# linto-ai/ssak

Measured on AMD Instinct MI355X. Metric: utterances/sec (16 kHz, 10 s) Wav2Vec2-base CTC train step, higher is better.
Workload: dtype bf16; 1 GPU; Wav2Vec2-base CTC fine-tune step, bf16, synthetic 10 s @16 kHz utterances (BASELINE.json configs[1]; DP over xGMI for n_gpus>1 = configs[2]); per_gpu_batch=32, global_batch=32, samples_per_utt=160000, frames=499, frozen_feature_encoder=True, regularisers=script defaults (dropout/layerdrop/specaugment on), parallelism=dp1

## Files before the change

ssak_amd/csrc/kernels.h:

```cpp
#pragma once
#include "common.h"

enum : int {
  PROF_ATTN_FWD = 0, PROF_ATTN_BWD, PROF_LN_FWD, PROF_LN_BWD, PROF_CONV0, PROF_ADAMW, PROF_SUMSQ, PROF_CTC, PROF_WAVE_NORM,
  PROF_ROWWISE, PROF_POSCONV_W, PROF_SOFTMAX, PROF_POSCONV_DIRECT, PROF_POSCONV_WGRAD, PROF_LOGMEL,
  PROF_CLASS_SLOTS
};
constexpr int PROF_MAX_SLOTS = 128;
int ssak_prof_register(const char* name, int bound);
bool ssak_prof_wanted(int slot, hipStream_t st);
class ProfScope {
 public:
  ProfScope(int slot, double work, hipStream_t st);
  ~ProfScope();
  ProfScope(const ProfScope&) = delete;
  ProfScope& operator=(const ProfScope&) = delete;

 private:
  hipStream_t st_;
  hipEvent_t e0_ = nullptr;
  int slot_;
  double work_;
  bool on_;
};

struct DropSpec {
  uint64_t seed = 0;
  uint32_t stream = 0;
  float p = 0.f;
};

struct ReduceJob {
  const float* partial;
  float* out;
  long stride;
  int slots, ncols;
};
struct ReduceSink {
  static constexpr int CAP = 32;
  ReduceJob jobs[CAP];
  int n = 0;
  bool push(const float* partial, long stride, int slots, int ncols, float* out) {
    if (n >= CAP) return false;
    jobs[n++] = ReduceJob{partial, out, stride, slots, ncols};
    return true;
  }
};
extern thread_local ReduceSink* g_reduce_sink;
int k_reduce_flush(ReduceSink& sink, hipStream_t st);

template <typename T>
int k_layernorm_fwd_t(const T* y, const T* res, const float* gamma, const float* beta, T* r_out, T* out,
                      float* mean, float* rstd, int M, int C, float eps, const DropSpec& pre, const DropSpec& post,
                      hipStream_t st, const DropSpec& mid = DropSpec(), bool post_gelu = false);
template <typename T>
int k_layernorm_bwd_t(const T* g1, const T* g2, const T* r, const float* mean, const float* rstd,
                      const float* gamma, const T* g_res, T* dr, T* dy, float* dgamma, float* dbeta,
                      float* partial , int M, int C, const DropSpec& pre, const DropSpec& post,
                      hipStream_t st, const DropSpec& mid = DropSpec(), float* dy_colsum = nullptr ,
                      const float* post_gelu_beta = nullptr );
#ifndef SSAK_LN_BWD_BLOCKS
#define SSAK_LN_BWD_BLOCKS 768
#endif
#ifndef SSAK_LN_FWD_BLOCKS
#define SSAK_LN_FWD_BLOCKS 768
#endif
constexpr int LN_FWD_BLOCKS = SSAK_LN_FWD_BLOCKS;
constexpr int LN_BWD_BLOCKS = SSAK_LN_BWD_BLOCKS;
template <typename T>
int k_softmax_fwd_t(const T* S, T* P, T* Pd, const int32_t* klens, int rows, int cols, int ld,
                    int rows_per_batch, const DropSpec& drop, hipStream_t st);
template <typename T>
int k_softmax_bwd_t(const T* dPd, const T* P, T* dS, int rows, int cols, int ld, const DropSpec& drop,
                    hipStream_t st);
template <typename T>
int k_colsum_t(const T* X, long ld, int M, int N, float* out, hipStream_t st, float* scratch = nullptr, size_t scratch_floats = 0,
               const uint8_t* rowmask = nullptr, const int32_t* flens = nullptr, int F = 0);
int k_cast_f32_bf16(const float* in, bf16* out, long n, hipStream_t st);
template <typename T>
int k_specaug_fwd_t(T* h, const uint8_t* mask, const int32_t* flens, const float* embed, int B, int F, int C,
                    hipStream_t st);
template <typename T>
int k_specaug_bwd_t(T* dh, const uint8_t* mask, const int32_t* flens, float* dembed, int B, int F, int C,
                    hipStream_t st, float* scratch = nullptr, size_t scratch_floats = 0);
template <typename T>
int k_gelu_grad_mul_t(const T* dy, const T* pre, T* out, long n, hipStream_t st);
template <typename T>
int k_add_t(const T* a, const T* b, T* out, long n, hipStream_t st);
int k_layernorm_fwd(const bf16* y, const bf16* res, const float* gamma, const float* beta, bf16* r_out, bf16* out,
                    float* mean, float* rstd, int M, int C, float eps, const DropSpec& pre, const DropSpec& post,
                    hipStream_t st, const DropSpec& mid = DropSpec(), bool post_gelu = false);
int k_layernorm_bwd(const bf16* g1, const bf16* g2, const bf16* r, const float* mean, const float* rstd,
                    const float* gamma, const bf16* g_res, bf16* dr, bf16* dy, float* dgamma, float* dbeta,
                    float* partial, int M, int C, const DropSpec& pre, const DropSpec& post,
                    hipStream_t st, const DropSpec& mid = DropSpec(), float* dy_colsum = nullptr,
                    const float* post_gelu_beta = nullptr);
int k_colsum(const bf16* X, long ld, int M, int N, float* out, hipStream_t st, float* scratch = nullptr, size_t scratch_floats = 0,
             const uint8_t* rowmask = nullptr, const int32_t* flens = nullptr, int F = 0);

size_t k_conv0_stats_doubles(int B, int T0, int C);
template <typename T>
int k_conv0_gn_gelu_t(const float* x, const float* w, const float* gamma, const float* beta, T* out, double* stats,
                      int B, int Tn, int T0, int C, int ksize, int stride, hipStream_t st, bool raw_input = false);
size_t k_conv0_wgrad_scratch_floats(int B, int C, int ksize);
template <typename DT>
int k_conv0_wgrad_t(const DT* d, const float* x, float* dw, float* scratch, int B, int T, int T0, int C, int ksize, int stride,
                  hipStream_t st);
template <typename T>
int k_conv0_bias_t(const float* x, const float* w, const float* bias, T* out, int B, int Tn, int T0, int C, int ksize,
                   int stride, hipStream_t st);
template <typename T_>
int k_col2im_t(const T_* dxcol, T_* dx, int B, int Tin, int Tout, int C, int k, int s, hipStream_t st);
int k_sum_slabs(const float* slabs, int nb, long n, float* out, hipStream_t st);
size_t k_conv0_bwd_scratch_floats(int B, int T0, int C);
template <typename DT>
int k_conv0_gn_gelu_bwd_t(const float* x, const float* w, const float* gamma, const float* beta, const DT* dy,
                        const double* sums, float* scratch, float* dw, float* dgamma, float* dbeta, int B, int T, int T0, int C,
                        hipStream_t st);
template <typename T>
int k_conv_weight_rearrange_t(const float* w, T* out, int Co, int Ci, int k, hipStream_t st);
template <typename T>
int k_posconv_prepare_t(const float* g, const float* v, T* w_fwd, T* w_bwd, float* norms, int H, int G, int K,
                        hipStream_t st);
int k_posconv_weight_bwd(const float* dw, const float* g, const float* v, const float* norms, float* dg, float* dv,
                         int H, int G, int K, hipStream_t st);
template <typename T>
int k_posconv_pack_t(const T* h, T* pg, int B, int F, int H, int G, int K, hipStream_t st);

bool k_attn_adapter_supported(int H, int A);
template <typename T>
int k_attn_adapter_fwd_t(const T* y, const T* res, const float* ln_g, const float* ln_b, const T* w1, const float* b1, const T* w2,
                         const float* b2, const float* next_g, const float* next_b, T* r_out, T* out, float* mean, float* rstd, int M,
                         int H, int A, float eps_adapter, float eps_next, hipStream_t st);

bool k_attention_supported(int H, int nh);
int k_attention_fwd(const bf16* qkv, bf16* ctx, float* lse, const int32_t* klens, int B, int F, int nh, int H,
                    const DropSpec& drop, hipStream_t st);
size_t k_attention_bwd_bias_floats(int B, int F, int H);
int k_attention_bwd(const bf16* qkv, const bf16* ctx, const float* lse, const int32_t* klens, const bf16* dctx, float* delta,
                    bf16* dqkv, int B, int F, int nh, int H, const DropSpec& drop, int mode , hipStream_t st,
                    float* bias_part = nullptr, float* bias_grad = nullptr);
int k_colsum_rows(const float* partial, int slots, int N, float* out, hipStream_t st);

bool k_posconv_direct_supported(int H, int G, int K);
int k_posconv_frag_weights(const bf16* w, bf16* wfrag, int H, int G, int K, hipStream_t st);
int k_posconv_direct(const bf16* x, long rows_per_group, int row0, const bf16* w, const float* bias, bf16* out, bf16* pre, int B, int F,
                     int H, int G, int K, int gelu, hipStream_t st);

size_t k_posconv_wgrad_scratch_floats(int H, int G, int K);
int k_posconv_wgrad_direct(const bf16* x, const bf16* dy, long rows_per_group, long rows, int lead, float* dwf, float* scratch, int H, int G,
                           int K, hipStream_t st);

template <typename T_>
int k_mel_to_cl_t(const float* mel, T_* cl, int B, int C, int T, int RS, int lead, hipStream_t st);
template <typename T_>
int k_add_rowvec_t(const T_* x, const T_* pos, T_* out, int B, int F, int H, hipStream_t st);
template <typename T_>
int k_copy_rows_padded_t(const T_* src, T_* dst, int B, int F, int RS, int H, hipStream_t st);
template <typename T_>
int k_col2im_k3s2_t(const T_* dxcol, const T_* pre, T_* out, int B, int F, int Tin, int RS1, int H, hipStream_t st);
int k_conv_wgrad_unrearrange(const float* dwr, float* g, int Co, int Ci, int k, hipStream_t st);

int k_sumsq(const float* g, long n, float* out , float* partial, hipStream_t st, bool add = false );
int k_adamw(float* p, const float* g, float* m, float* v, bf16* shadow, long n, const float* gnorm_sq, float max_norm,
            float grad_scale, float lr, float beta1, float beta2, float eps, float wd, int step, hipStream_t st);

int ssak_gemm_p8_launch(const void* params, int bm, int a_km, int b_km, hipStream_t st);
int k_transpose_bf16_batched(int n, const bf16* const* src, bf16* const* dst, const int* R, const int* C, hipStream_t st);

int ssak_gemm_ticket_slot(hipStream_t st, int** out);
bool ssak_gemm_p4_supports(const void* params, int bm, int a_km, int b_km);
int ssak_gemm_p4_launch(const void* params, int bm, int b_km, hipStream_t st);
int ssak_gemm_p8bd_launch(const void* params, int bm, hipStream_t st);
size_t k_gemm_fragment_b_bytes(int N, int K);
int k_gemm_fragment_b_batched(int n, const void* const* B, const long* ldb, const int* N, const int* K, const int* b_km, void* const* out,
                              hipStream_t st);
int ssak_gemm_p8_launch_grouped(const void* params, int n, const void* const* A, const void* const* B, void* const* C, const int* M,
                                const int* N, const long* lda, const long* ldb, const long* ldc, const uint32_t* ext_a,
                                const uint32_t* ext_b, int a_km, int b_km, hipStream_t st);
```

ssak_amd/csrc/norm_act.hip:

```cpp
#include <algorithm>
#include <type_traits>

#include "common.h"
#include "kernels.h"

namespace {

SSAK_DEFINE_DROP_TABLE

constexpr int ROW_THREADS = 256;
template <int VEC>
__device__ __forceinline__ void load_colmul(uint32_t (&cm)[VEC], int col0) {
#pragma unroll
  for (int k = 0; k < VEC; k += 4) {
    const uint4 t = *reinterpret_cast<const uint4*>(g_drop_colmul.v + col0 + k);
    cm[k] = t.x, cm[k + 1] = t.y, cm[k + 2] = t.z, cm[k + 3] = t.w;
  }
}

template <typename T, int VEC>
using ChunkT = typename std::conditional<VEC == 8, Chunk8<T>, Chunk4<T>>::type;
template <typename T, int VEC>
__device__ __forceinline__ ChunkT<T, VEC> f_to_chunk(const float* f) {
  if constexpr (VEC == 8) return f_to_chunk8<T>(f);
  else return f_to_chunk4<T>(f);
}

template <typename T>
struct LnFwdParams {
  const T* y;
  const T* res;
  const float* gamma;
  const float* beta;
  T* r_out;
  T* out;
  float* mean;
  float* rstd;
  int M, C;
  float eps;
  uint64_t seed;
  uint32_t pre_stream, pre_thresh, post_stream, post_thresh;
  float pre_scale, post_scale;
  uint32_t mid_stream, mid_thresh;
  float mid_scale;
  int post_gelu;
};

template <typename T, int NCH>
__global__ __launch_bounds__(ROW_THREADS) void ln_fwd_kernel(const LnFwdParams<T> p) {
  const int lane = threadIdx.x & 63;
  const int row = blockIdx.x * (ROW_THREADS / 64) + (threadIdx.x >> 6);
  if (row >= p.M) return;
  const int nch = p.C >> 3;
  float v[NCH][8];
  float s = 0.f;
  const bool any_drop = (p.pre_thresh | p.mid_thresh | p.post_thresh) != 0;
  const uint32_t rk_pre = p.pre_thresh ? drop_rowkey(p.seed, p.pre_stream, (uint64_t)row) : 1u;
  const uint32_t rk_mid = p.mid_thresh ? drop_rowkey(p.seed, p.mid_stream, (uint64_t)row) : 1u;
  const uint32_t rk_post = p.post_thresh ? drop_rowkey(p.seed, p.post_stream, (uint64_t)row) : 1u;
  const uint32_t thi_pre = p.pre_thresh << 16, thi_mid = p.mid_thresh << 16, thi_post = p.post_thresh << 16;
  uint32_t cm[NCH][8];
#pragma unroll
  for (int i = 0; i < NCH; ++i) {
    const int ch = lane + 64 * i;
#pragma unroll
    for (int k = 0; k < 8; ++k) v[i][k] = 0.f;
    if (ch < nch) {
      const size_t o = (size_t)row * p.C + ch * 8;
      if (any_drop) load_colmul<8>(cm[i], ch * 8);
      if (p.y) {
        chunk_to_f(ld8<T>(p.y + o), v[i]);
        if (p.pre_thresh) {
#pragma unroll
          for (int k = 0; k < 8; ++k) v[i][k] = drop_keep(rk_pre, cm[i][k], thi_pre) ? v[i][k] * p.pre_scale : 0.f;
        }
      }
      if (p.res) {
        float r[8];
        chunk_to_f(ld8<T>(p.res + o), r);
#pragma unroll
        for (int k = 0; k < 8; ++k) v[i][k] += r[k];
      }
      if (p.mid_thresh) {
#pragma unroll
        for (int k = 0; k < 8; ++k) v[i][k] = drop_keep(rk_mid, cm[i][k], thi_mid) ? v[i][k] * p.mid_scale : 0.f;
      }
      if (p.r_out) {
        const Chunk8<T> q = f_to_chunk8<T>(v[i]);
        st8<T>(p.r_out + o, q);
        chunk_to_f(q, v[i]);
      }
#pragma unroll
      for (int k = 0; k < 8; ++k) s += v[i][k];
    }
  }
  if (!p.out) return;
  const float mean = wave_sum(s) / (float)p.C;
  float q2 = 0.f;
#pragma unroll
  for (int i = 0; i < NCH; ++i)
    if (lane + 64 * i < nch) {
#pragma unroll
      for (int k = 0; k < 8; ++k) {
        const float d = v[i][k] - mean;
        q2 += d * d;
      }
    }
  const float rstd = rsqrtf(wave_sum(q2) / (float)p.C + p.eps);
  if (lane == 0 && p.mean) {
    p.mean[row] = mean;
    p.rstd[row] = rstd;
  }
#pragma unroll
  for (int i = 0; i < NCH; ++i) {
    const int ch = lane + 64 * i;
    if (ch < nch) {
      const size_t o = (size_t)row * p.C + ch * 8;
      float g[8], b[8], w[8];
      *reinterpret_cast<float4*>(g) = *reinterpret_cast<const float4*>(p.gamma + ch * 8);
      *reinterpret_cast<float4*>(g + 4) = *reinterpret_cast<const float4*>(p.gamma + ch * 8 + 4);
      *reinterpret_cast<float4*>(b) = *reinterpret_cast<const float4*>(p.beta + ch * 8);
      *reinterpret_cast<float4*>(b + 4) = *reinterpret_cast<const float4*>(p.beta + ch * 8 + 4);
#pragma unroll
      for (int k = 0; k < 8; ++k) {
        w[k] = (v[i][k] - mean) * rstd * g[k] + b[k];
        if (p.post_gelu) w[k] = gelu_s<T>(w[k]);
        if (p.post_thresh) w[k] = drop_keep(rk_post, cm[i][k], thi_post) ? w[k] * p.post_scale : 0.f;
      }
      st8<T>(p.out + o, f_to_chunk8<T>(w));
    }
  }
}

template <typename T, int NCH, int VEC, int SPEC>
__global__ __launch_bounds__(ROW_THREADS) void ln_fwd_rows_kernel(const LnFwdParams<T> p) {
  using VecT = ChunkT<T, VEC>;
  constexpr bool HAS_Y = (SPEC & 1) != 0, HAS_RES = (SPEC & 2) != 0, D_PRE = (SPEC & 4) != 0, D_MID = (SPEC & 8) != 0,
                 D_POST = (SPEC & 16) != 0, HAS_ROUT = (SPEC & 32) != 0, DROP = (SPEC & 28) != 0;
  const int lane = threadIdx.x & 63;
  const int wid = blockIdx.x * (ROW_THREADS / 64) + (threadIdx.x >> 6);
  const int rstep = gridDim.x * (ROW_THREADS / 64);
  float gm[NCH][VEC], bt[NCH][VEC];
  uint32_t cm[DROP ? NCH : 1][VEC];
#pragma unroll
  for (int i = 0; i < NCH; ++i) {
    const int c0 = (lane + 64 * i) * VEC;
#pragma unroll
    for (int k = 0; k < VEC; ++k) gm[i][k] = p.gamma[c0 + k], bt[i][k] = p.beta[c0 + k];
    if (DROP) load_colmul<VEC>(cm[i], c0);
  }
  const uint32_t thi_pre = p.pre_thresh << 16, thi_mid = p.mid_thresh << 16, thi_post = p.post_thresh << 16;
  const float inv_c = 1.f / (float)p.C;
  VecT ny[NCH], nr[NCH];
  auto fetch = [&](int row) {
#pragma unroll
    for (int i = 0; i < NCH; ++i) {
      const size_t o = (size_t)row * p.C + (lane + 64 * i) * VEC;
      if (HAS_Y) ny[i] = *reinterpret_cast<const VecT*>(p.y + o);
      if (HAS_RES) nr[i] = *reinterpret_cast<const VecT*>(p.res + o);
    }
  };
  if (wid < p.M) fetch(wid);
  for (int row = wid; row < p.M; row += rstep) {
    VecT cy[NCH], cr[NCH];
#pragma unroll
    for (int i = 0; i < NCH; ++i) cy[i] = ny[i], cr[i] = nr[i];
    if (row + rstep < p.M) fetch(row + rstep);
    const uint32_t rk_pre = D_PRE ? drop_rowkey(p.seed, p.pre_stream, (uint64_t)row) : 1u;
    const uint32_t rk_mid = D_MID ? drop_rowkey(p.seed, p.mid_stream, (uint64_t)row) : 1u;
    const uint32_t rk_post = D_POST ? drop_rowkey(p.seed, p.post_stream, (uint64_t)row) : 1u;
    float v[NCH][VEC];
    float s = 0.f;
#pragma unroll
    for (int i = 0; i < NCH; ++i) {
      const size_t o = (size_t)row * p.C + (lane + 64 * i) * VEC;
#pragma unroll
      for (int k = 0; k < VEC; ++k) v[i][k] = 0.f;
      if (HAS_Y) {
        chunk_to_f(cy[i], v[i]);
        if (D_PRE) {
#pragma unroll
          for (int k = 0; k < VEC; ++k) v[i][k] = drop_keep(rk_pre, cm[DROP ? i : 0][k], thi_pre) ? v[i][k] * p.pre_scale : 0.f;
        }
      }
      if (HAS_RES) {
        float r[VEC];
        chunk_to_f(cr[i], r);
#pragma unroll
        for (int k = 0; k < VEC; ++k) v[i][k] += r[k];
      }
      if (D_MID) {
#pragma unroll
        for (int k = 0; k < VEC; ++k) v[i][k] = drop_keep(rk_mid, cm[DROP ? i : 0][k], thi_mid) ? v[i][k] * p.mid_scale : 0.f;
      }
      if (HAS_ROUT) {
        const VecT q = f_to_chunk<T, VEC>(v[i]);
        *reinterpret_cast<VecT*>(p.r_out + o) = q;
        chunk_to_f(q, v[i]);
      }
#pragma unroll
      for (int k = 0; k < VEC; ++k) s += v[i][k];
    }
    const float mean = wave_sum(s) * inv_c;
    float q2 = 0.f;
#pragma unroll
    for (int i = 0; i < NCH; ++i)
#pragma unroll
      for (int k = 0; k < VEC; ++k) {
        const float d = v[i][k] - mean;
        q2 += d * d;
      }
    const float rstd = rsqrtf(wave_sum(q2) * inv_c + p.eps);
    if (lane == 0 && p.mean) {
      p.mean[row] = mean;
      p.rstd[row] = rstd;
    }
#pragma unroll
    for (int i = 0; i < NCH; ++i) {
      const size_t o = (size_t)row * p.C + (lane + 64 * i) * VEC;
      float w[VEC];
#pragma unroll
      for (int k = 0; k < VEC; ++k) {
        w[k] = (v[i][k] - mean) * rstd * gm[i][k] + bt[i][k];
        if (D_POST) w[k] = drop_keep(rk_post, cm[DROP ? i : 0][k], thi_post) ? w[k] * p.post_scale : 0.f;
      }
      *reinterpret_cast<VecT*>(p.out + o) = f_to_chunk<T, VEC>(w);
    }
  }
}

template <typename T>
struct LnBwdParams {
  const T* g1;
  const T* g2;
  const T* r;
  const float* mean;
  const float* rstd;
  const float* gamma;
  const T* g_res;
  T* dr;
  T* dy;
  float* dgamma;
  float* dbeta;
  float* partial;
  float* dy_colsum;
  const float* beta;
  int M, C;
  uint64_t seed;
  uint32_t pre_stream, pre_thresh, post_stream, post_thresh;
  float pre_scale, post_scale;
  int rows_per_wave;
  uint32_t mid_stream, mid_thresh;
  float mid_scale;
};

template <typename T, int NCH, int VEC, bool PGELU, bool DROP, int SPEC = -1>
__global__ __launch_bounds__(ROW_THREADS) void ln_bwd_kernel(const LnBwdParams<T> p) {
  using VecT = ChunkT<T, VEC>;
  __shared__ float red[3][ROW_THREADS / 64][NCH * VEC][64];
  constexpr bool S = SPEC >= 0;
  const bool has_dy = S ? (SPEC & 1) != 0 : p.dy != nullptr;
  const bool d_pre = S ? (SPEC & 2) != 0 : (DROP && p.pre_thresh != 0);
  const bool d_mid = S ? (SPEC & 4) != 0 : (DROP && p.mid_thresh != 0);
  const bool d_post = S ? (SPEC & 8) != 0 : (DROP && p.post_thresh != 0);
  const bool has_g2 = S ? (SPEC & 16) != 0 : p.g2 != nullptr;
  const bool has_gres = S ? (SPEC & 32) != 0 : p.g_res != nullptr;
  constexpr bool PF_GRES = S && (SPEC & 32) != 0 && (SPEC & 16) == 0;
  const int lane = threadIdx.x & 63, wave = threadIdx.x >> 6;
  const int nch = p.C / VEC;
  const int wid = blockIdx.x * (ROW_THREADS / 64) + wave;
  float ag[NCH][VEC], ab[NCH][VEC], gm[NCH][VEC], ay[NCH][VEC], bt[PGELU ? NCH : 1][VEC];
  uint32_t cm[DROP ? NCH : 1][VEC];
#pragma unroll
  for (int i = 0; i < NCH; ++i) {
    const int ch = lane + 64 * i;
#pragma unroll
    for (int k = 0; k < VEC; ++k) {
      ag[i][k] = 0.f;
      ab[i][k] = 0.f;
      ay[i][k] = 0.f;
      gm[i][k] = (S || ch < nch) ? p.gamma[ch * VEC + k] : 0.f;
      if (PGELU) bt[i][k] = (ch < nch) ? p.beta[ch * VEC + k] : 0.f;
    }
    if (DROP && (S || ch < nch)) load_colmul<VEC>(cm[i], ch * VEC);
  }
  const uint32_t thi_pre = p.pre_thresh << 16, thi_mid = p.mid_thresh << 16, thi_post = p.post_thresh << 16;
  const int rstep = gridDim.x * (ROW_THREADS / 64);
  VecT ra[NCH], rb[NCH], rx[NCH], re[NCH];
  float mean_n = 0.f, rstd_n = 0.f;
  auto fetch = [&](int row) {
    mean_n = p.mean[row];
    rstd_n = p.rstd[row];
#pragma unroll
    for (int i = 0; i < NCH; ++i) {
      const int ch = lane + 64 * i;
      if (S || ch < nch) {
        const size_t o = (size_t)row * p.C + ch * VEC;
        ra[i] = *reinterpret_cast<const VecT*>(p.g1 + o);
        if (has_g2) rb[i] = *reinterpret_cast<const VecT*>(p.g2 + o);
        rx[i] = *reinterpret_cast<const VecT*>(p.r + o);
        if (PF_GRES) re[i] = *reinterpret_cast<const VecT*>(p.g_res + o);
      }
    }
  };
  if (wid < p.M) fetch(wid);
  for (int row = wid; row < p.M; row += rstep) {
    const float mean = mean_n, rstd = rstd_n;
    uint32_t rk_pre = 1u, rk_mid = 1u, rk_post = 1u;
    if (DROP) {
      if (d_pre) rk_pre = drop_rowkey(p.seed, p.pre_stream, (uint64_t)row);
      if (d_mid) rk_mid = drop_rowkey(p.seed, p.mid_stream, (uint64_t)row);
      if (d_post) rk_post = drop_rowkey(p.seed, p.post_stream, (uint64_t)row);
    }
    float dyv[NCH][VEC], xh[NCH][VEC];
    float s1 = 0.f, s2 = 0.f;
    VecT ca[NCH], cb[NCH], cx[NCH], ce[NCH];
#pragma unroll
    for (int i = 0; i < NCH; ++i) {
      ca[i] = ra[i];
      cb[i] = rb[i];
      cx[i] = rx[i];
      ce[i] = re[i];
    }
    if (row + rstep < p.M) fetch(row + rstep);
#pragma unroll
    for (int i = 0; i < NCH; ++i) {
      const int ch = lane + 64 * i;
#pragma unroll
      for (int k = 0; k < VEC; ++k) {
        dyv[i][k] = 0.f;
        xh[i][k] = 0.f;
      }
      if (S || ch < nch) {
        float a[VEC], x[VEC];
        chunk_to_f(ca[i], a);
        if (has_g2) {
          float b2[VEC];
          chunk_to_f(cb[i], b2);
#pragma unroll
          for (int k = 0; k < VEC; ++k) a[k] += b2[k];
        }
        chunk_to_f(cx[i], x);
#pragma unroll
        for (int k = 0; k < VEC; ++k) {
          if (d_post) a[k] = drop_keep(rk_post, cm[DROP ? i : 0][k], thi_post) ? a[k] * p.post_scale : 0.f;
          xh[i][k] = (x[k] - mean) * rstd;
          if (PGELU) a[k] *= gelu_grad_s<T>(fmaf(xh[i][k], gm[i][k], bt[PGELU ? i : 0][k]));
          ag[i][k] += a[k] * xh[i][k];
          ab[i][k] += a[k];
          dyv[i][k] = a[k] * gm[i][k];
          s1 += dyv[i][k];
          s2 += dyv[i][k] * xh[i][k];
        }
      }
    }
    s1 = wave_sum(s1) / (float)p.C;
    s2 = wave_sum(s2) / (float)p.C;
#pragma unroll
    for (int i = 0; i < NCH; ++i) {
      const int ch = lane + 64 * i;
      if (S || ch < nch) {
        const size_t o = (size_t)row * p.C + ch * VEC;
        float d[VEC];
#pragma unroll
        for (int k = 0; k < VEC; ++k) d[k] = rstd * (dyv[i][k] - s1 - xh[i][k] * s2);
        if (has_gres) {
          float e[VEC];
          if (PF_GRES) chunk_to_f(ce[i], e);
          else chunk_to_f(*reinterpret_cast<const VecT*>(p.g_res + o), e);
#pragma unroll
          for (int k = 0; k < VEC; ++k) d[k] += e[k];
        }
        if (d_mid) {
#pragma unroll
          for (int k = 0; k < VEC; ++k) d[k] = drop_keep(rk_mid, cm[DROP ? i : 0][k], thi_mid) ? d[k] * p.mid_scale : 0.f;
        }
        *reinterpret_cast<VecT*>(p.dr + o) = f_to_chunk<T, VEC>(d);
        if (has_dy) {
#pragma unroll
          for (int k = 0; k < VEC; ++k) {
            d[k] = (!d_pre || drop_keep(rk_pre, cm[DROP ? i : 0][k], thi_pre)) ? d[k] * p.pre_scale : 0.f;
            ay[i][k] += d[k];
          }
          *reinterpret_cast<VecT*>(p.dy + o) = f_to_chunk<T, VEC>(d);
        }
      }
    }
  }
#pragma unroll
  for (int i = 0; i < NCH; ++i)
#pragma unroll
    for (int k = 0; k < VEC; ++k) {
      red[0][wave][i * VEC + k][lane] = ag[i][k];
      red[1][wave][i * VEC + k][lane] = ab[i][k];
      red[2][wave][i * VEC + k][lane] = ay[i][k];
    }
  lds_barrier();
  for (int e = threadIdx.x; e < NCH * VEC * 64; e += ROW_THREADS) {
    const int slot = e >> 6, ln = e & 63;
    const int i = slot / VEC, k = slot % VEC;
    const int col = (ln + 64 * i) * VEC + k;
    if (col < p.C) {
      float sg = 0.f, sb = 0.f, sy = 0.f;
#pragma unroll
      for (int w = 0; w < ROW_THREADS / 64; ++w) {
        sg += red[0][w][slot][ln];
        sb += red[1][w][slot][ln];
        sy += red[2][w][slot][ln];
      }
      p.partial[((size_t)blockIdx.x * 3) * p.C + col] = sg;
      p.partial[((size_t)blockIdx.x * 3 + 1) * p.C + col] = sb;
      p.partial[((size_t)blockIdx.x * 3 + 2) * p.C + col] = sy;
    }
  }
}

__global__ __launch_bounds__(1024) void ln_bwd_finalize_kernel(const float* __restrict__ partial, int nblk, int C,
                                                               float* __restrict__ dgamma, float* __restrict__ dbeta,
                                                               float* __restrict__ dy_colsum) {
  __shared__ float red[16][65];
  const int cx = threadIdx.x & 63, ry = threadIdx.x >> 6;
  const int e = blockIdx.x * 64 + cx;
  const int planes = dy_colsum ? 3 : 2;
  float s = 0.f;
  if (e < planes * C) {
    const int which = e / C, col = e % C;
#pragma unroll 8
    for (int b = ry; b < nblk; b += 16) s += partial[((size_t)b * 3 + which) * C + col];
  }
  red[ry][cx] = s;
  __syncthreads();
  if (ry == 0 && e < planes * C) {
    float t = 0.f;
#pragma unroll
    for (int r = 0; r < 16; ++r) t += red[r][cx];
    const int which = e / C, col = e % C;
    float* dst = which == 0 ? dgamma : which == 1 ? dbeta : dy_colsum;
    dst[col] += t;
  }
}

struct ReduceTable {
  ReduceJob jobs[ReduceSink::CAP];
  int first_block[ReduceSink::CAP + 1];
  int n;
};
__global__ __launch_bounds__(1024) void reduce_jobs_kernel(const ReduceTable t) {
  __shared__ float red[16][65];
  int j = 0;
  for (int k = 1; k < t.n; ++k) j = (int)blockIdx.x >= t.first_block[k] ? k : j;
  const ReduceJob& q = t.jobs[j];
  const int cx = threadIdx.x & 63, ry = threadIdx.x >> 6;
  const int n = ((int)blockIdx.x - t.first_block[j]) * 64 + cx;
  float s = 0.f;
  if (n < q.ncols) {
    int k = ry;
    for (; k + 15 * 16 < q.slots; k += 16 * 16) {
      float v[16];
#pragma unroll
      for (int u = 0; u < 16; ++u) v[u] = q.partial[(long)(k + 16 * u) * q.stride + n];
#pragma unroll
      for (int u = 0; u < 16; ++u) s += v[u];
    }
    for (; k < q.slots; k += 16) s += q.partial[(long)k * q.stride + n];
  }
  red[ry][cx] = s;
  __syncthreads();
  if (ry == 0 && n < q.ncols) {
    float v = 0.f;
#pragma unroll
    for (int r = 0; r < 16; ++r) v += red[r][cx];
    q.out[n] += v;
  }
}

template <typename T>
struct SoftmaxParams {
  const T* S;
  T* P;
  T* Pd;
  const int32_t* klens;
  int rows, cols, ld, rows_per_batch;
  uint64_t seed;
  uint32_t stream, thresh;
  float scale;
};

template <typename T, int NCH>
__global__ __launch_bounds__(ROW_THREADS) void softmax_fwd_kernel(const SoftmaxParams<T> p) {
  const int lane = threadIdx.x & 63;
  const int row = blockIdx.x * (ROW_THREADS / 64) + (threadIdx.x >> 6);
  if (row >= p.rows) return;
  const int kl = p.klens ? min(p.klens[row / p.rows_per_batch], p.cols) : p.cols;
  const int nch = p.ld >> 3;
  float v[NCH][8];
  float mx = -INFINITY;
#pragma unroll
  for (int i = 0; i < NCH; ++i) {
    const int ch = lane + 64 * i;
#pragma unroll
    for (int k = 0; k < 8; ++k) v[i][k] = -INFINITY;
    if (ch < nch) {
      float f[8];
      chunk_to_f(ld8<T>(p.S + (size_t)row * p.ld + ch * 8), f);
#pragma unroll
      for (int k = 0; k < 8; ++k) {
        v[i][k] = (ch * 8 + k < kl) ? f[k] : -INFINITY;
        mx = fmaxf(mx, v[i][k]);
      }
    }
  }
  mx = wave_max(mx);
  float sum = 0.f;
#pragma unroll
  for (int i = 0; i < NCH; ++i)
#pragma unroll
    for (int k = 0; k < 8; ++k) {
      v[i][k] = (v[i][k] == -INFINITY) ? 0.f : __expf(v[i][k] - mx);
      sum += v[i][k];
    }
  const float tot = wave_sum(sum);
  const float inv = tot > 0.f ? 1.f / tot : 0.f;
#pragma unroll
  for (int i = 0; i < NCH; ++i) {
    const int ch = lane + 64 * i;
    if (ch < nch) {
      const size_t o = (size_t)row * p.ld + ch * 8;
      float pr[8];
#pragma unroll
      for (int k = 0; k < 8; ++k) pr[k] = v[i][k] * inv;
      st8<T>(p.P + o, f_to_chunk8<T>(pr));
      if (p.Pd) {
        const uint32_t rs = drop_rowkey(p.seed, p.stream, (uint64_t)row);
#pragma unroll
        for (int k = 0; k < 8; ++k) pr[k] = (!p.thresh || drop_keep(rs, drop_colmul((uint32_t)(ch * 8 + k)), p.thresh << 16)) ? pr[k] * p.scale : 0.f;
        st8<T>(p.Pd + o, f_to_chunk8<T>(pr));
      }
    }
  }
}
// ... 380 lines not shown
  SSAK_LAUNCH_CHECK();
  return SSAK_OK;
}

template <typename T>
int k_specaug_fwd_t(T* h, const uint8_t* mask, const int32_t* flens, const float* embed, int B, int F, int C,
                    hipStream_t st) {
  if (!mask && !flens) return SSAK_OK;
  ProfScope prof_scope(PROF_ROWWISE, (double)B * F * 1.0, st);
  specaug_fwd_kernel<T><<<B * F, 128, 0, st>>>(h, mask, flens, embed, B * F, F, C);
  SSAK_LAUNCH_CHECK();
  return SSAK_OK;
}

template <typename T>
int k_specaug_bwd_t(T* dh, const uint8_t* mask, const int32_t* flens, float* dembed, int B, int F, int C,
                    hipStream_t st, float* scratch, size_t scratch_floats) {
  if (!mask && !flens) return SSAK_OK;
  if (mask && dembed)
    if (int rc = k_colsum_t<T>(dh, C, B * F, C, dembed, st, scratch, scratch_floats, mask, flens, F)) return rc;
  specaug_bwd_kernel<T><<<B * F, 128, 0, st>>>(dh, mask, flens, dembed, B * F, F, C);
  SSAK_LAUNCH_CHECK();
  return SSAK_OK;
}

template <typename T>
int k_gelu_grad_mul_t(const T* dy, const T* pre, T* out, long n, hipStream_t st) {
  SSAK_REQUIRE((n & 7) == 0, "gelu_grad_mul: n must be a multiple of 8");
  ProfScope prof_scope(PROF_ROWWISE, (double)n * 6.0, st);
  gelu_grad_mul_kernel<T><<<min(4096, ssak_cdiv(n / 8, 256)), 256, 0, st>>>(dy, pre, out, n / 8);
  SSAK_LAUNCH_CHECK();
  return SSAK_OK;
}

template <typename T>
int k_add_t(const T* a, const T* b, T* out, long n, hipStream_t st) {
  SSAK_REQUIRE((n & 7) == 0, "add: n must be a multiple of 8");
  ProfScope prof_scope(PROF_ROWWISE, (double)n * 6.0, st);
  add_kernel<T><<<min(4096, ssak_cdiv(n / 8, 256)), 256, 0, st>>>(a, b, out, n / 8);
  SSAK_LAUNCH_CHECK();
  return SSAK_OK;
}

#define SSAK_INSTANTIATE_ROW_KERNELS(T)                                                                                           \
  template int k_layernorm_fwd_t<T>(const T*, const T*, const float*, const float*, T*, T*, float*, float*, int, int, float,      \
                                    const DropSpec&, const DropSpec&, hipStream_t, const DropSpec&, bool);                        \
  template int k_layernorm_bwd_t<T>(const T*, const T*, const T*, const float*, const float*, const float*, const T*, T*, T*,     \
                                    float*, float*, float*, int, int, const DropSpec&, const DropSpec&, hipStream_t,              \
                                    const DropSpec&, float*, const float*);                                                       \
  template int k_softmax_fwd_t<T>(const T*, T*, T*, const int32_t*, int, int, int, int, const DropSpec&, hipStream_t);            \
  template int k_softmax_bwd_t<T>(const T*, const T*, T*, int, int, int, const DropSpec&, hipStream_t);                           \
  template int k_colsum_t<T>(const T*, long, int, int, float*, hipStream_t, float*, size_t, const uint8_t*, const int32_t*, int); \
  template int k_specaug_fwd_t<T>(T*, const uint8_t*, const int32_t*, const float*, int, int, int, hipStream_t);                  \
  template int k_specaug_bwd_t<T>(T*, const uint8_t*, const int32_t*, float*, int, int, int, hipStream_t, float*, size_t);        \
  template int k_gelu_grad_mul_t<T>(const T*, const T*, T*, long, hipStream_t);                                                   \
  template int k_add_t<T>(const T*, const T*, T*, long, hipStream_t);
SSAK_INSTANTIATE_ROW_KERNELS(bf16)
SSAK_INSTANTIATE_ROW_KERNELS(float)

int k_layernorm_fwd(const bf16* y, const bf16* res, const float* gamma, const float* beta, bf16* r_out, bf16* out,
                    float* mean, float* rstd, int M, int C, float eps, const DropSpec& pre, const DropSpec& post,
                    hipStream_t st, const DropSpec& mid, bool post_gelu) {
  return k_layernorm_fwd_t<bf16>(y, res, gamma, beta, r_out, out, mean, rstd, M, C, eps, pre, post, st, mid, post_gelu);
}
int k_layernorm_bwd(const bf16* g1, const bf16* g2, const bf16* r, const float* mean, const float* rstd,
                    const float* gamma, const bf16* g_res, bf16* dr, bf16* dy, float* dgamma, float* dbeta,
                    float* partial, int M, int C, const DropSpec& pre, const DropSpec& post, hipStream_t st,
                    const DropSpec& mid, float* dy_colsum, const float* post_gelu_beta) {
  return k_layernorm_bwd_t<bf16>(g1, g2, r, mean, rstd, gamma, g_res, dr, dy, dgamma, dbeta, partial, M, C, pre, post, st, mid,
                                 dy_colsum, post_gelu_beta);
}
int k_colsum(const bf16* X, long ld, int M, int N, float* out, hipStream_t st, float* scratch, size_t scratch_floats,
             const uint8_t* rowmask, const int32_t* flens, int F) {
  return k_colsum_t<bf16>(X, ld, M, N, out, st, scratch, scratch_floats, rowmask, flens, F);
}

__global__ void debug_dropout_mask_kernel(uint64_t seed, uint32_t stream, uint32_t thresh, long rows, int cols, uint8_t* keep) {
  const long i = (long)blockIdx.x * blockDim.x + threadIdx.x;
  if (i >= rows * cols) return;
  keep[i] = (!thresh || keep_bit(seed, stream, (uint64_t)(i / cols), (uint32_t)(i % cols), thresh)) ? 1 : 0;
}
extern "C" int ssak_debug_dropout_mask(uint64_t seed, uint32_t site, float p, long rows, int cols, uint8_t* keep, float* scale_out ,
                                       void* stream) {
  SSAK_REQUIRE(keep && rows > 0 && cols > 0, "debug_dropout_mask: bad arguments");
  const long n = rows * cols;
  debug_dropout_mask_kernel<<<(unsigned)((n + 255) / 256), 256, 0, (hipStream_t)stream>>>(seed, site, thresh_of(p), rows, cols, keep);
  SSAK_LAUNCH_CHECK();
  if (scale_out) *scale_out = scale_of(p);
  return SSAK_OK;
}
extern "C" int ssak_debug_attention_dropout_mask(uint64_t seed, uint32_t site, float p, int B, int nh, int F, uint8_t* keep,
                                                 void* stream) {
  SSAK_REQUIRE(keep && B > 0 && nh > 0 && F > 0, "debug_attention_dropout_mask: bad arguments");
  return ssak_debug_dropout_mask(seed, site, p, (long)B * nh * F, F, keep, nullptr, stream);
}

namespace {
DropSpec debug_site(uint64_t seed, uint32_t site, float p) {
  DropSpec d;
  d.seed = seed;
  d.stream = site;
  d.p = p;
  return d;
}
bool debug_p_ok(float p) { return p >= 0.f && p < 1.f; }

template <typename T>
__global__ void debug_gelu_kernel(const float* __restrict__ x, long n, float* __restrict__ y, float* __restrict__ dydx) {
  const long i = (long)blockIdx.x * blockDim.x + threadIdx.x;
  if (i >= n) return;
  if (y) y[i] = gelu_s<T>(x[i]);
  if (dydx) dydx[i] = gelu_grad_s<T>(x[i]);
}
}

extern "C" int ssak_debug_layernorm_fwd(const void* y, const void* res, const float* gamma, const float* beta, void* r_out, void* out,
                                        float* mean, float* rstd, int M, int C, float eps, uint64_t seed, uint32_t pre_site, float pre_p,
                                        uint32_t mid_site, float mid_p, uint32_t post_site, float post_p, int post_gelu, int dtype,
                                        void* stream) {
  SSAK_REQUIRE(dtype == 0 || dtype == 1, "debug_layernorm_fwd: dtype %d (0 bf16, 1 fp32)", dtype);
  SSAK_REQUIRE(M > 0 && C > 0 && (C & 7) == 0 && C <= 1536, "debug_layernorm_fwd: M=%d C=%d (C a multiple of 8, <= 1536)", M, C);
  SSAK_REQUIRE(y || res, "debug_layernorm_fwd: neither y nor res");
  SSAK_REQUIRE(out || r_out, "debug_layernorm_fwd: neither out nor r_out");
  SSAK_REQUIRE(!out || (gamma && beta), "debug_layernorm_fwd: out needs gamma and beta");
  SSAK_REQUIRE(!mean == !rstd, "debug_layernorm_fwd: mean and rstd go together");
  SSAK_REQUIRE(out || (!mean && !post_gelu && post_p == 0.f), "debug_layernorm_fwd: statistics, GELU and post-dropout need out");
  SSAK_REQUIRE(debug_p_ok(pre_p) && debug_p_ok(mid_p) && debug_p_ok(post_p), "debug_layernorm_fwd: p outside [0, 1)");
  SSAK_REQUIRE(y || pre_p == 0.f, "debug_layernorm_fwd: pre-dropout without y");
  const DropSpec pre = debug_site(seed, pre_site, pre_p), mid = debug_site(seed, mid_site, mid_p), post = debug_site(seed, post_site, post_p);
  const hipStream_t st = (hipStream_t)stream;
  if (dtype == 0)
    return k_layernorm_fwd_t<bf16>((const bf16*)y, (const bf16*)res, gamma, beta, (bf16*)r_out, (bf16*)out, mean, rstd, M, C, eps, pre,
                                   post, st, mid, post_gelu != 0);
  return k_layernorm_fwd_t<float>((const float*)y, (const float*)res, gamma, beta, (float*)r_out, (float*)out, mean, rstd, M, C, eps,
                                  pre, post, st, mid, post_gelu != 0);
}

extern "C" int ssak_layernorm_fwd(const void* y, const void* res, const float* gamma, const float* beta, void* r_out, void* out, int M, int C,
                                  float eps, int dtype, void* stream) {
  SSAK_REQUIRE(dtype == 0 || dtype == 1, "layernorm_fwd: dtype %d (0 bf16, 1 fp32)", dtype);
  SSAK_REQUIRE(M > 0 && C > 0 && (C & 7) == 0 && C <= 1536, "layernorm_fwd: M=%d C=%d (C a multiple of 8, <= 1536)", M, C);
  SSAK_REQUIRE(y || res, "layernorm_fwd: neither y nor res");
  SSAK_REQUIRE(out || r_out, "layernorm_fwd: neither out nor r_out");
  SSAK_REQUIRE(!out || (gamma && beta), "layernorm_fwd: out needs gamma and beta");
  const DropSpec none;
  const hipStream_t st = (hipStream_t)stream;
  if (dtype == 0)
    return k_layernorm_fwd_t<bf16>((const bf16*)y, (const bf16*)res, gamma, beta, (bf16*)r_out, (bf16*)out, nullptr, nullptr, M, C, eps, none,
                                   none, st);
  return k_layernorm_fwd_t<float>((const float*)y, (const float*)res, gamma, beta, (float*)r_out, (float*)out, nullptr, nullptr, M, C, eps, none,
                                  none, st);
}

extern "C" size_t ssak_debug_layernorm_bwd_workspace_bytes(int C) { return C > 0 ? (size_t)LN_BWD_BLOCKS * 3 * C * sizeof(float) : 0; }

extern "C" int ssak_debug_layernorm_bwd(const void* g1, const void* g2, const void* r, const float* mean, const float* rstd,
                                        const float* gamma, const void* g_res, void* dr, void* dy, float* dgamma, float* dbeta,
                                        float* dy_colsum, const float* post_gelu_beta, int M, int C, uint64_t seed, uint32_t pre_site,
                                        float pre_p, uint32_t mid_site, float mid_p, uint32_t post_site, float post_p, int queued,
                                        int dtype, void* workspace, size_t workspace_bytes, void* stream) {
  SSAK_REQUIRE(dtype == 0 || dtype == 1, "debug_layernorm_bwd: dtype %d (0 bf16, 1 fp32)", dtype);
  SSAK_REQUIRE(M > 0 && C > 0 && (C & 7) == 0 && C <= 1536, "debug_layernorm_bwd: M=%d C=%d (C a multiple of 8, <= 1536)", M, C);
  SSAK_REQUIRE(g1 && r && mean && rstd && gamma && dr && dgamma && dbeta, "debug_layernorm_bwd: null operand");
  SSAK_REQUIRE(!dy_colsum || dy, "debug_layernorm_bwd: dy_colsum needs dy");
  SSAK_REQUIRE(debug_p_ok(pre_p) && debug_p_ok(mid_p) && debug_p_ok(post_p), "debug_layernorm_bwd: p outside [0, 1)");
  SSAK_REQUIRE(workspace && workspace_bytes >= ssak_debug_layernorm_bwd_workspace_bytes(C), "debug_layernorm_bwd: workspace too small");
  const DropSpec pre = debug_site(seed, pre_site, pre_p), mid = debug_site(seed, mid_site, mid_p), post = debug_site(seed, post_site, post_p);
  const hipStream_t st = (hipStream_t)stream;
  ReduceSink sink;
  ReduceSink* const saved = g_reduce_sink;
  if (queued) g_reduce_sink = &sink;
  int rc;
  if (dtype == 0)
    rc = k_layernorm_bwd_t<bf16>((const bf16*)g1, (const bf16*)g2, (const bf16*)r, mean, rstd, gamma, (const bf16*)g_res, (bf16*)dr,
                                 (bf16*)dy, dgamma, dbeta, (float*)workspace, M, C, pre, post, st, mid, dy_colsum, post_gelu_beta);
  else
    rc = k_layernorm_bwd_t<float>((const float*)g1, (const float*)g2, (const float*)r, mean, rstd, gamma, (const float*)g_res,
                                  (float*)dr, (float*)dy, dgamma, dbeta, (float*)workspace, M, C, pre, post, st, mid, dy_colsum,
                                  post_gelu_beta);
  g_reduce_sink = saved;
  if (rc != SSAK_OK || !queued) return rc;
  SSAK_REQUIRE(sink.n == (dy_colsum ? 3 : 2), "debug_layernorm_bwd: %d column sums queued", sink.n);
  return k_reduce_flush(sink, st);
}

extern "C" int ssak_debug_softmax_fwd(const void* S, void* P, void* Pd, const int32_t* klens, int rows, int cols, int ld,
                                      int rows_per_batch, uint64_t seed, uint32_t site, float p, int dtype, void* stream) {
  SSAK_REQUIRE(dtype == 0 || dtype == 1, "debug_softmax_fwd: dtype %d (0 bf16, 1 fp32)", dtype);
  SSAK_REQUIRE(rows > 0 && cols > 0 && ld >= cols && (ld & 7) == 0 && ld <= 1536, "debug_softmax_fwd: rows=%d cols=%d ld=%d (ld >= cols, "
               "a multiple of 8, <= 1536)", rows, cols, ld);
  SSAK_REQUIRE(S && P, "debug_softmax_fwd: null operand");
  SSAK_REQUIRE(!klens || rows_per_batch > 0, "debug_softmax_fwd: klens needs rows_per_batch > 0");
  SSAK_REQUIRE(debug_p_ok(p) && (Pd || p == 0.f), "debug_softmax_fwd: p outside [0, 1) or dropout without Pd");
  const DropSpec d = debug_site(seed, site, p);
  if (dtype == 0)
    return k_softmax_fwd_t<bf16>((const bf16*)S, (bf16*)P, (bf16*)Pd, klens, rows, cols, ld, rows_per_batch, d, (hipStream_t)stream);
  return k_softmax_fwd_t<float>((const float*)S, (float*)P, (float*)Pd, klens, rows, cols, ld, rows_per_batch, d, (hipStream_t)stream);
}

extern "C" int ssak_debug_softmax_bwd(const void* dPd, const void* P, void* dS, int rows, int cols, int ld, uint64_t seed, uint32_t site,
                                      float p, int dtype, void* stream) {
  SSAK_REQUIRE(dtype == 0 || dtype == 1, "debug_softmax_bwd: dtype %d (0 bf16, 1 fp32)", dtype);
  SSAK_REQUIRE(rows > 0 && cols > 0 && ld >= cols && (ld & 7) == 0 && ld <= 1536, "debug_softmax_bwd: rows=%d cols=%d ld=%d (ld >= cols, "
               "a multiple of 8, <= 1536)", rows, cols, ld);
  SSAK_REQUIRE(dPd && P && dS, "debug_softmax_bwd: null operand");
  SSAK_REQUIRE(debug_p_ok(p), "debug_softmax_bwd: p outside [0, 1)");
  const DropSpec d = debug_site(seed, site, p);
  if (dtype == 0) return k_softmax_bwd_t<bf16>((const bf16*)dPd, (const bf16*)P, (bf16*)dS, rows, cols, ld, d, (hipStream_t)stream);
  return k_softmax_bwd_t<float>((const float*)dPd, (const float*)P, (float*)dS, rows, cols, ld, d, (hipStream_t)stream);
}

extern "C" int ssak_debug_gelu(const float* x, long n, float* y, float* dydx, int dtype, void* stream) {
  SSAK_REQUIRE(dtype == 0 || dtype == 1, "debug_gelu: dtype %d (0 bf16, 1 fp32)", dtype);
  SSAK_REQUIRE(x && n > 0 && (y || dydx), "debug_gelu: bad arguments");
  const unsigned grid = (unsigned)((n + 255) / 256);
  if (dtype == 0) debug_gelu_kernel<bf16><<<grid, 256, 0, (hipStream_t)stream>>>(x, n, y, dydx);
  else debug_gelu_kernel<float><<<grid, 256, 0, (hipStream_t)stream>>>(x, n, y, dydx);
  SSAK_LAUNCH_CHECK();
  return SSAK_OK;
}
```

Measured before the change: 2255 utterances/sec.

## Double-buffer LayerNorm row prefetch and shrink backward grid to fewer blocks

Rewrites the LayerNorm forward and backward row loops as a two-stage ping-pong pipeline. Each loop alternates two register buffers, uses scheduling barriers and asm register pins so the next row's loads stay in flight while the current row is computed, and reads the per-row mean/rstd through the constant address space. The backward grid drops from 768 to 256 blocks, which cuts the number of per-block column partials to reduce but gives fewer waves to hide latency. The extra buffers raise register pressure, and the last prefetch is clamped to the final row, so that row is loaded redundantly.

```diff
diff --git a/ssak_amd/csrc/kernels.h b/ssak_amd/csrc/kernels.h
--- a/ssak_amd/csrc/kernels.h
+++ b/ssak_amd/csrc/kernels.h
@@ -60,7 +60,7 @@
                       hipStream_t st, const DropSpec& mid = DropSpec(), float* dy_colsum = nullptr ,
                       const float* post_gelu_beta = nullptr );
 #ifndef SSAK_LN_BWD_BLOCKS
-#define SSAK_LN_BWD_BLOCKS 768
+#define SSAK_LN_BWD_BLOCKS 256
 #endif
 #ifndef SSAK_LN_FWD_BLOCKS
 #define SSAK_LN_FWD_BLOCKS 768
diff --git a/ssak_amd/csrc/norm_act.hip b/ssak_amd/csrc/norm_act.hip
--- a/ssak_amd/csrc/norm_act.hip
+++ b/ssak_amd/csrc/norm_act.hip
@@ -16,6 +16,20 @@
     const uint4 t = *reinterpret_cast<const uint4*>(g_drop_colmul.v + col0 + k);
     cm[k] = t.x, cm[k + 1] = t.y, cm[k + 2] = t.z, cm[k + 3] = t.w;
   }
+}
+
+__device__ __forceinline__ float ld_wave_uniform(const float* q) {
+  return *(const __attribute__((address_space(4))) float*)q;
+}
+
+template <typename C>
+__device__ __forceinline__ void pin_chunk(C& c) {
+  static_assert(sizeof(C) % 4 == 0, "chunks are whole dwords");
+  uint32_t w[sizeof(C) / 4];
+  __builtin_memcpy(w, &c, sizeof(C));
+#pragma unroll
+  for (size_t k = 0; k < sizeof(C) / 4; ++k) asm volatile("" : "+v"(w[k]));
+  __builtin_memcpy(&c, w, sizeof(C));
 }
 
 template <typename T, int VEC>
@@ -138,8 +152,9 @@
   constexpr bool HAS_Y = (SPEC & 1) != 0, HAS_RES = (SPEC & 2) != 0, D_PRE = (SPEC & 4) != 0, D_MID = (SPEC & 8) != 0,
                  D_POST = (SPEC & 16) != 0, HAS_ROUT = (SPEC & 32) != 0, DROP = (SPEC & 28) != 0;
   const int lane = threadIdx.x & 63;
-  const int wid = blockIdx.x * (ROW_THREADS / 64) + (threadIdx.x >> 6);
+  const int wid = blockIdx.x * (ROW_THREADS / 64) + __builtin_amdgcn_readfirstlane(threadIdx.x >> 6);
   const int rstep = gridDim.x * (ROW_THREADS / 64);
+  if (wid >= p.M) return;
   float gm[NCH][VEC], bt[NCH][VEC];
   uint32_t cm[DROP ? NCH : 1][VEC];
 #pragma unroll
@@ -151,21 +166,20 @@
   }
   const uint32_t thi_pre = p.pre_thresh << 16, thi_mid = p.mid_thresh << 16, thi_post = p.post_thresh << 16;
   const float inv_c = 1.f / (float)p.C;
-  VecT ny[NCH], nr[NCH];
-  auto fetch = [&](int row) {
+  auto fetch = [&](VecT(&fy)[NCH], VecT(&fr)[NCH], int row) {
 #pragma unroll
     for (int i = 0; i < NCH; ++i) {
       const size_t o = (size_t)row * p.C + (lane + 64 * i) * VEC;
-      if (HAS_Y) ny[i] = *reinterpret_cast<const VecT*>(p.y + o);
-      if (HAS_RES) nr[i] = *reinterpret_cast<const VecT*>(p.res + o);
+      if (HAS_Y) fy[i] = *reinterpret_cast<const VecT*>(p.y + o);
+      if (HAS_RES) fr[i] = *reinterpret_cast<const VecT*>(p.res + o);
     }
   };
-  if (wid < p.M) fetch(wid);
-  for (int row = wid; row < p.M; row += rstep) {
-    VecT cy[NCH], cr[NCH];
-#pragma unroll
-    for (int i = 0; i < NCH; ++i) cy[i] = ny[i], cr[i] = nr[i];
-    if (row + rstep < p.M) fetch(row + rstep);
+  auto do_row = [&](VecT(&cy)[NCH], VecT(&cr)[NCH], int row) {
+#pragma unroll
+    for (int i = 0; i < NCH; ++i) {
+      if (HAS_Y) pin_chunk(cy[i]);
+      if (HAS_RES) pin_chunk(cr[i]);
+    }
     const uint32_t rk_pre = D_PRE ? drop_rowkey(p.seed, p.pre_stream, (uint64_t)row) : 1u;
     const uint32_t rk_mid = D_MID ? drop_rowkey(p.seed, p.mid_stream, (uint64_t)row) : 1u;
     const uint32_t rk_post = D_POST ? drop_rowkey(p.seed, p.post_stream, (uint64_t)row) : 1u;
@@ -226,7 +240,21 @@
       }
       *reinterpret_cast<VecT*>(p.out + o) = f_to_chunk<T, VEC>(w);
     }
-  }
+  };
+  const int last = p.M - 1;
+  VecT y0[NCH], r0[NCH], y1[NCH], r1[NCH];
+  fetch(y0, r0, wid);
+  __builtin_amdgcn_s_waitcnt(0x0f70);
+  int row = wid;
+  for (; row + rstep < p.M; row += 2 * rstep) {
+    fetch(y1, r1, row + rstep);
+    __builtin_amdgcn_sched_barrier(0);
+    do_row(y0, r0, row);
+    fetch(y0, r0, min(row + 2 * rstep, last));
+    __builtin_amdgcn_sched_barrier(0);
+    do_row(y1, r1, row + rstep);
+  }
+  if (row < p.M) do_row(y0, r0, row);
 }
 
 template <typename T>
@@ -268,7 +296,7 @@
   constexpr bool PF_GRES = S && (SPEC & 32) != 0 && (SPEC & 16) == 0;
   const int lane = threadIdx.x & 63, wave = threadIdx.x >> 6;
   const int nch = p.C / VEC;
-  const int wid = blockIdx.x * (ROW_THREADS / 64) + wave;
+  const int wid = blockIdx.x * (ROW_THREADS / 64) + __builtin_amdgcn_readfirstlane(wave);
   float ag[NCH][VEC], ab[NCH][VEC], gm[NCH][VEC], ay[NCH][VEC], bt[PGELU ? NCH : 1][VEC];
   uint32_t cm[DROP ? NCH : 1][VEC];
 #pragma unroll
@@ -286,26 +314,35 @@
   }
   const uint32_t thi_pre = p.pre_thresh << 16, thi_mid = p.mid_thresh << 16, thi_post = p.post_thresh << 16;
   const int rstep = gridDim.x * (ROW_THREADS / 64);
-  VecT ra[NCH], rb[NCH], rx[NCH], re[NCH];
-  float mean_n = 0.f, rstd_n = 0.f;
-  auto fetch = [&](int row) {
-    mean_n = p.mean[row];
-    rstd_n = p.rstd[row];
+  struct RowOps {
+    VecT a[NCH], b[NCH], x[NCH], e[NCH];
+    float mean, rstd;
+  };
+  auto fetch = [&](RowOps& f, int row) {
+    f.mean = ld_wave_uniform(p.mean + row);
+    f.rstd = ld_wave_uniform(p.rstd + row);
 #pragma unroll
     for (int i = 0; i < NCH; ++i) {
       const int ch = lane + 64 * i;
       if (S || ch < nch) {
         const size_t o = (size_t)row * p.C + ch * VEC;
-        ra[i] = *reinterpret_cast<const VecT*>(p.g1 + o);
-        if (has_g2) rb[i] = *reinterpret_cast<const VecT*>(p.g2 + o);
-        rx[i] = *reinterpret_cast<const VecT*>(p.r + o);
-        if (PF_GRES) re[i] = *reinterpret_cast<const VecT*>(p.g_res + o);
+        f.a[i] = *reinterpret_cast<const VecT*>(p.g1 + o);
+        if (has_g2) f.b[i] = *reinterpret_cast<const VecT*>(p.g2 + o);
+        f.x[i] = *reinterpret_cast<const VecT*>(p.r + o);
+        if (PF_GRES) f.e[i] = *reinterpret_cast<const VecT*>(p.g_res + o);
       }
     }
   };
-  if (wid < p.M) fetch(wid);
-  for (int row = wid; row < p.M; row += rstep) {
-    const float mean = mean_n, rstd = rstd_n;
+  auto do_row = [&](RowOps& c, int row) {
+#pragma unroll
+    for (int i = 0; i < NCH; ++i)
+      if (S || lane + 64 * i < nch) {
+        pin_chunk(c.a[i]);
+        if (has_g2) pin_chunk(c.b[i]);
+        pin_chunk(c.x[i]);
+        if (PF_GRES) pin_chunk(c.e[i]);
+      }
+    const float mean = c.mean, rstd = c.rstd;
     uint32_t rk_pre = 1u, rk_mid = 1u, rk_post = 1u;
     if (DROP) {
       if (d_pre) rk_pre = drop_rowkey(p.seed, p.pre_stream, (uint64_t)row);
@@ -314,15 +351,6 @@
     }
     float dyv[NCH][VEC], xh[NCH][VEC];
     float s1 = 0.f, s2 = 0.f;
-    VecT ca[NCH], cb[NCH], cx[NCH], ce[NCH];
-#pragma unroll
-    for (int i = 0; i < NCH; ++i) {
-      ca[i] = ra[i];
-      cb[i] = rb[i];
-      cx[i] = rx[i];
-      ce[i] = re[i];
-    }
-    if (row + rstep < p.M) fetch(row + rstep);
 #pragma unroll
     for (int i = 0; i < NCH; ++i) {
       const int ch = lane + 64 * i;
@@ -333,14 +361,14 @@
       }
       if (S || ch < nch) {
         float a[VEC], x[VEC];
-        chunk_to_f(ca[i], a);
+        chunk_to_f(c.a[i], a);
         if (has_g2) {
           float b2[VEC];
-          chunk_to_f(cb[i], b2);
+          chunk_to_f(c.b[i], b2);
 #pragma unroll
           for (int k = 0; k < VEC; ++k) a[k] += b2[k];
         }
-        chunk_to_f(cx[i], x);
+        chunk_to_f(c.x[i], x);
 #pragma unroll
         for (int k = 0; k < VEC; ++k) {
           if (d_post) a[k] = drop_keep(rk_post, cm[DROP ? i : 0][k], thi_post) ? a[k] * p.post_scale : 0.f;
@@ -366,7 +394,7 @@
         for (int k = 0; k < VEC; ++k) d[k] = rstd * (dyv[i][k] - s1 - xh[i][k] * s2);
         if (has_gres) {
           float e[VEC];
-          if (PF_GRES) chunk_to_f(ce[i], e);
+          if (PF_GRES) chunk_to_f(c.e[i], e);
           else chunk_to_f(*reinterpret_cast<const VecT*>(p.g_res + o), e);
 #pragma unroll
           for (int k = 0; k < VEC; ++k) d[k] += e[k];
@@ -386,6 +414,22 @@
         }
       }
     }
+  };
+  if (wid < p.M) {
+    const int last = p.M - 1;
+    RowOps o0, o1;
+    fetch(o0, wid);
+    __builtin_amdgcn_s_waitcnt(0x0f70);
+    int row = wid;
+    for (; row + rstep < p.M; row += 2 * rstep) {
+      fetch(o1, row + rstep);
+      __builtin_amdgcn_sched_barrier(0);
+      do_row(o0, row);
+      fetch(o0, min(row + 2 * rstep, last));
+      __builtin_amdgcn_sched_barrier(0);
+      do_row(o1, row + rstep);
+    }
+    if (row < p.M) do_row(o0, row);
   }
 #pragma unroll
   for (int i = 0; i < NCH; ++i)
@@ -1072,7 +1116,9 @@
                                   none, st);
 }
 
-extern "C" size_t ssak_debug_layernorm_bwd_workspace_bytes(int C) { return C > 0 ? (size_t)LN_BWD_BLOCKS * 3 * C * sizeof(float) : 0; }
+extern "C" size_t ssak_debug_layernorm_bwd_workspace_bytes(int C) {
+  return C > 0 ? (size_t)std::max(LN_BWD_BLOCKS, 768) * 3 * C * sizeof(float) : 0;
+}
 
 extern "C" int ssak_debug_layernorm_bwd(const void* g1, const void* g2, const void* r, const float* mean, const float* rstd,
                                         const float* gamma, const void* g_res, void* dr, void* dy, float* dgamma, float* dbeta,
```

Result: no change. 2265 utterances/sec (median of 6 runs) (+0.4%).
